# diegoferigo/gym-ignition

Hardware: AMD Instinct MI355X
Metric: env·steps/sec (whole node) at N parallel worlds; obs max-abs-err vs DART (higher is better)
Workload: dtype f32

## Files before the change

### gym-ignition_amd/csrc/vecenv_kernel.hip

```cpp
#include <cstdlib>
#include <type_traits>

#include "baked_models.hpp"
#include "chain_dyn.hpp"
#include "kernels.hpp"
#include "rng.hpp"

namespace mw {
namespace dev {

__constant__ constexpr baked::CartpoleBlock kCartpoleDev = {{MW_BAKED_CARTPOLE_INIT}};
__constant__ constexpr baked::PendulumBlock kPendulumDev = {{MW_BAKED_PENDULUM_INIT}};

template <int BAKED>
__device__ __forceinline__ const ChainF* model_params(const ChainF* P) {
    if constexpr (BAKED == baked::kCartpoleId) return reinterpret_cast<const ChainF*>(&kCartpoleDev);
    else if constexpr (BAKED == baked::kPendulumId) return reinterpret_cast<const ChainF*>(&kPendulumDev);
    else return P;
}

struct VecTail {
    float* obs;
    float* reward;
    uint8_t* done;
    float* term_obs;
    int32_t T_steps;
    int32_t max_steps;
    int32_t reward_cart_at_center;
    uint32_t seed_lo, seed_hi;
    uint32_t world_offset;
    float force_mag;
    float x_factor;
    float hi[4];
};
struct VecTailRand : VecTail {
    int32_t randomize;
    float mass_lo, mass_hi;
    float g_mean, g_std;
    float gdir[3];
    float* rmass;
    float* rgz;
};
template <bool RAND, bool GENERIC>
struct VecArgs : std::conditional_t<RAND, VecTailRand, VecTail> {};
template <bool RAND>
struct VecArgs<RAND, true> : std::conditional_t<RAND, VecTailRand, VecTail> {
    const ChainF* P;
};
static_assert(sizeof(VecArgs<true, true>) <= 136, "the step kernel's kernargs stay within 192 bytes");

template <class A>
__device__ __forceinline__ void fetch_now(const A& a) {
    static_assert(sizeof(A) % 4 == 0);
    uint32_t v[sizeof(A) / 4];
    __builtin_memcpy(v, &a, sizeof(A));
#pragma unroll
    for (unsigned k = 0; k < sizeof(A) / 4; ++k) asm volatile("" ::"s"(v[k]));
}

constexpr float kPi = 3.14159265358979323846f;

template <int N, int KIND, bool FOLD = false, class TT>
__device__ __forceinline__ void task_reset(const TT& T, uint32_t w, uint32_t episode,
                                           float (&q)[N], float (&qd)[N]) {
    uint32_t r[4];
    philox(T.seed_lo, T.seed_hi, w, episode, r);
    const auto unif = [](uint32_t x, float lo, float hi) {
        if constexpr (FOLD) return unif_folded(x, lo, hi);
        else return dev::unif(x, lo, hi);
    };
    if constexpr (KIND == 0 || KIND == 1) {
        q[0] = unif(r[0], -0.05f, 0.05f); qd[0] = unif(r[1], -0.05f, 0.05f);
        q[1] = unif(r[2], -0.05f, 0.05f); qd[1] = unif(r[3], -0.05f, 0.05f);
    } else if constexpr (KIND == 2) {
        q[1] = kPi - unif(r[0], -60.f, 60.f) * (kPi / 180.f);
        q[0] = unif(r[1], -0.05f, 0.05f); qd[0] = unif(r[2], -0.05f, 0.05f);
        qd[1] = unif(r[3], -0.05f, 0.05f);
    } else {
        const float c = unif(r[0], -1.f, 1.f), s = unif(r[1], -1.f, 1.f);
        q[0] = atan2f(s, c);
        qd[0] = unif(r[2], -10.f, 10.f);
    }
}

template <int N, int KIND>
__device__ __forceinline__ void task_obs(const float (&q)[N], const float (&qd)[N], float (&o)[4]) {
    if constexpr (KIND == 3) {
        float s, c;
        sincosf(q[0], &s, &c);
        o[0] = c; o[1] = s; o[2] = qd[0]; o[3] = 0.f;
    } else {
        o[0] = q[0]; o[1] = qd[0]; o[2] = q[1]; o[3] = qd[1];
    }
}

template <int KIND, bool ABS = false, class TT>
__device__ __forceinline__ bool task_done(const TT& T, const float (&o)[4]) {
    constexpr int no = (KIND == 3) ? 3 : 4;
    bool inside = true;
#pragma unroll
    for (int k = 0; k < no; ++k) {
        if constexpr (ABS) inside = inside & (fabsf(o[k]) <= T.hi[k]);
        else inside = inside & (o[k] >= -T.hi[k]) & (o[k] <= T.hi[k]);
    }
    return !inside;
}

template <int N, int KIND, class TT>
__device__ __forceinline__ float task_reward(const TT& T, const float (&q)[N], const float (&qd)[N],
                                             const float (&o)[4], bool done) {
#pragma clang fp contract(off)
    if constexpr (KIND == 0 || KIND == 1) {
        float r = done ? 0.f : 1.f;
        if (T.reward_cart_at_center)
            r = r - 0.10f * fabsf(o[0]) - 0.10f * fabsf(o[1]) -
                10.0f * (o[0] >= T.x_factor * 2.4f ? 1.f : 0.f);
        return r;
    } else if constexpr (KIND == 2) {
        return (cosf(q[1]) + 1.f) * 0.5f - 0.1f * qd[0] * qd[0] -
               10.0f * (q[0] >= T.x_factor * 2.4f ? 1.f : 0.f);
    } else {
        const float cost = (done ? 100.f : 0.f) + q[0] * q[0] + 0.1f * qd[0] * qd[0];
        return -cost;
    }
}

template <int N, class TT>
__device__ __forceinline__ Dyn<N> sample_dyn(const ChainF* __restrict__ P, const TT& T, uint32_t w,
                                             uint32_t episode, float& gz_out) {
    Dyn<N> D = nominal_dyn<N>(P);
    gz_out = 0.f;
    if (T.randomize & kRandMass) {
#pragma unroll
        for (int b = 0; b < (N + 3) / 4; ++b) {
            uint32_t r[4];
            philox(T.seed_lo, T.seed_hi, w, episode, r, 1u + static_cast<uint32_t>(b));
#pragma unroll
            for (int k = 0; k < 4; ++k)
                if (4 * b + k < N) D.m[4 * b + k] += fmaxf(unif(r[k], T.mass_lo, T.mass_hi), 0.f);
        }
    }
    if (T.randomize & kRandGravity) {
        uint32_t r[4];
        philox(T.seed_lo, T.seed_hi, w, episode, r, 8u);
        const float u1 = static_cast<float>((r[0] >> 8) + 1u) * (1.f / 16777216.f);
        const float u2 = static_cast<float>(r[1] >> 8) * (1.f / 16777216.f);
        const float z = sqrtf(-2.f * logf(u1)) * cosf(2.f * kPi * u2);
        const float gz = T.g_mean + T.g_std * z;
        D.g = {gz * T.gdir[0], gz * T.gdir[1], gz * T.gdir[2]};
        gz_out = gz;
    }
    return D;
}

template <int N, class TT, class VV>
__device__ __forceinline__ Dyn<N> load_dyn(const ChainF* __restrict__ P, const TT& T, const VV& V, int W, int w) {
    Dyn<N> D = nominal_dyn<N>(P);
    if (T.randomize & kRandMass) {
#pragma unroll
        for (int d = 0; d < N; ++d) D.m[d] = V.rmass[d * W + w];
    }
    if (T.randomize & kRandGravity) {
        const float gz = V.rgz[w];
        D.g = {gz * T.gdir[0], gz * T.gdir[1], gz * T.gdir[2]};
    }
    return D;
}

template <int N, class TT, class VV>
__device__ __forceinline__ void store_dyn(const TT& T, const VV& V, int W, int w, const Dyn<N>& D, float gz) {
    if (T.randomize & kRandMass) {
#pragma unroll
        for (int d = 0; d < N; ++d) V.rmass[d * W + w] = D.m[d];
    }
    if (T.randomize & kRandGravity) V.rgz[w] = gz;
}

template <bool OFF32, class E, class I>
__device__ __forceinline__ E* elem(E* base, I i) {
    if constexpr (OFF32) {
        using Byte = std::conditional_t<std::is_const_v<E>, const char, char>;
        return reinterpret_cast<E*>(reinterpret_cast<Byte*>(base) +
                                    static_cast<uint32_t>(i) * static_cast<uint32_t>(sizeof(E)));
    } else {
        return base + i;
    }
}

__device__ __forceinline__ int own_block(int w) {
    asm volatile("" : "+v"(w));
    return w;
}

template <int N, bool OFF32 = false>
__device__ __forceinline__ void store_state(float* __restrict__ sq, float* __restrict__ sqd, int W, int w,
                                            const float (&q)[N], const float (&qd)[N]) {
#pragma unroll
    for (int d = 0; d < N; ++d) {
        *elem<OFF32>(sq, d * W + w) = q[d];
        *elem<OFF32>(sqd, d * W + w) = qd[d];
    }
}

template <int NO>
__device__ __forceinline__ void store_obs(float* __restrict__ dst, const float (&o)[4]) {
    if constexpr (NO == 4) {
        *reinterpret_cast<float4*>(dst) = make_float4(o[0], o[1], o[2], o[3]);
    } else {
#pragma unroll
        for (int k = 0; k < NO; ++k) dst[k] = o[k];
    }
}


template <int N, int KIND>
__global__ void __launch_bounds__(256) vecenv_reset_kernel(const ChainF* __restrict__ P, TaskF T, SimDev S,
                                                           VecDev V, float* __restrict__ obs, int W) {
    const int w = blockIdx.x * blockDim.x + threadIdx.x;
    if (w >= W) return;
    float q[N], qd[N], o[4];
    if (T.randomize) {
        const uint32_t gw = T.world_offset + static_cast<uint32_t>(w);
        float gz;
        const Dyn<N> D = sample_dyn<N>(P, T, gw, 0u, gz);
        store_dyn<N>(T, V, W, w, D, gz);
    }
    task_reset<N, KIND>(T, T.world_offset + static_cast<uint32_t>(w), 0u, q, qd);
    task_obs<N, KIND>(q, qd, o);
    constexpr int NO = (KIND == 3) ? 3 : 4;
    store_obs<NO>(obs + static_cast<size_t>(w) * NO, o);
    store_state<N>(S.q, S.qd, W, w, q, qd);
    V.episode[w] = 0u;
    V.steps[w] = 0u;
}

constexpr int kHelpMaxWorlds = 64 * 256;
template <int N, int KIND, bool DUAL, bool CONS, bool ROLLOUT, int BAKED, bool RAND, int B, bool HELP = false,
          bool ONE = false>
__global__ void __launch_bounds__(256) vecenv_step_kernel(float* __restrict__ sq, float* __restrict__ sqd,
                                                          uint32_t* __restrict__ ep, uint32_t* __restrict__ st,
                                                          const void* __restrict__ actions, int W, float dt,
                                                          int substeps, int pgs_iters,
                                                          VecArgs<RAND, BAKED == 0> A) {
    static_assert(!HELP || (B == 64 && !ROLLOUT && !RAND), "the helper wave serves the closed-loop 64-world blocks");
    static_assert(!ONE || HELP, "the single-substep form exists for the helper-wave kernels");
    static_assert(static_cast<uint64_t>(kHelpMaxWorlds) * (N > 4 ? N : 4) * sizeof(float) < (1ull << 32),
                  "32-bit byte offsets cover every array of the HELP kernels");
    __shared__ float reset_lds[HELP ? 2 * N * B : 1];
    const int lane = HELP ? static_cast<int>(threadIdx.x) & (B - 1) : static_cast<int>(threadIdx.x);
    int w = blockIdx.x * B + lane;
    bool live = true;
    if constexpr (HELP) {
        live = w < W;
        w = live ? w : W - 1;
    } else {
        if (w >= W) return;
    }
    constexpr int NO = (KIND == 3) ? 3 : 4;
    using ActT = std::conditional_t<KIND == 0, int32_t, float>;
    float q[N], qd[N];
#pragma unroll
    for (int d = 0; d < N; ++d) {
        q[d] = *elem<HELP>(sq, d * W + w);
        qd[d] = *elem<HELP>(sqd, d * W + w);
    }
    const uint32_t episode0 = *elem<HELP>(ep, w);
    uint32_t episode = episode0;
    uint32_t steps = *elem<HELP>(st, w);
    ActT a0 = ActT(0);
    if constexpr (!ROLLOUT) a0 = *elem<HELP>(static_cast<const ActT*>(actions), w);
    fetch_now(A);
    float* __restrict__ obs = A.obs;
    float* __restrict__ reward = A.reward;
    uint8_t* __restrict__ done_out = A.done;
    float* __restrict__ term_obs = A.term_obs;
    const ChainF* __restrict__ P;
    if constexpr (BAKED == 0) P = A.P;
    else P = model_params<BAKED>(nullptr);
    uint8_t act[N];
    float vc[N];
#pragma unroll
    for (int d = 0; d < N; ++d) { act[d] = kActForce; vc[d] = 0.f; }
    Dyn<N> D;
    if constexpr (RAND) D = load_dyn<N>(P, A, A, W, w);
    if constexpr (HELP) {
        if (__builtin_amdgcn_readfirstlane(static_cast<int>(threadIdx.x)) >= B) {
            float rq[N], rqd[N];
            task_reset<N, KIND, true>(A, A.world_offset + static_cast<uint32_t>(w), episode0 + 1u, rq, rqd);
#pragma unroll
            for (int d = 0; d < N; ++d) {
                reset_lds[d * B + lane] = rq[d];
                reset_lds[(N + d) * B + lane] = rqd[d];
            }
            __syncthreads();
#pragma unroll
            for (int d = 0; d < N; ++d) asm volatile("" ::"v"(q[d]), "v"(qd[d]));
            asm volatile("" ::"v"(steps), "v"(a0));
            return;
        }
    }
    int ws = w;
    const int nsteps = ROLLOUT ? A.T_steps : 1;
    for (int t = 0; t < nsteps; ++t) {
        const size_t idx = static_cast<size_t>(t) * W + w;
        ActT a = a0;
        if constexpr (ROLLOUT) a = static_cast<const ActT*>(actions)[idx];
        float force;
        if constexpr (KIND == 0) {
            force = (a == 1) ? A.force_mag : -A.force_mag;
        } else {
            force = a;
        }
        const float e = P->b[0].effort;
        force = fminf(fmaxf(force, -e), e);
        float tau[N], qdd[N];
        if constexpr (ONE) {
#pragma unroll
            for (int d = 0; d < N; ++d) tau[d] = 0.f;
            tau[0] = force;
            substep<N, DUAL, CONS>(P, q, qd, tau, act, vc, dt, pgs_iters, qdd);
        } else {
            for (int s = 0; s < substeps; ++s) {
#pragma unroll
                for (int d = 0; d < N; ++d) tau[d] = 0.f;
                tau[0] = (s == 0) ? force : 0.f;
                if constexpr (RAND) substep_dyn<N, DUAL, CONS>(P, q, qd, tau, act, vc, dt, pgs_iters, qdd, D);
                else substep<N, DUAL, CONS>(P, q, qd, tau, act, vc, dt, pgs_iters, qdd);
            }
        }
        if constexpr (!ROLLOUT) asm volatile("" ::"v"(a0));
        float o[4];
        task_obs<N, KIND>(q, qd, o);
        const bool tdone = task_done<KIND, HELP>(A, o);
        const float rew = task_reward<N, KIND>(A, q, qd, o, tdone);
        if constexpr (!HELP) reward[idx] = rew;
        steps += 1u;
        const bool d_ = tdone || (A.max_steps > 0 && steps >= static_cast<uint32_t>(A.max_steps));
        if constexpr (HELP) {
            __syncthreads();
            if (!live) return;
            *elem<HELP>(reward, idx) = rew;
        }
        if constexpr (HELP) *elem<true>(done_out, idx) = d_ ? 1 : 0;
        else done_out[idx] = d_ ? 1 : 0;
        if (d_) {
            if constexpr (HELP) store_obs<NO>(elem<true>(term_obs, own_block(w) * NO), o);
            else store_obs<NO>(term_obs + idx * NO, o);
            episode += 1u;
            steps = 0u;
            if constexpr (RAND) {
                float gz;
                D = sample_dyn<N>(P, A, A.world_offset + static_cast<uint32_t>(w), episode, gz);
                store_dyn<N>(A, A, W, w, D, gz);
            }
            if constexpr (HELP) {
#pragma unroll
                for (int d = 0; d < N; ++d) {
                    q[d] = reset_lds[d * B + lane];
                    qd[d] = reset_lds[(N + d) * B + lane];
                }
            } else {
                task_reset<N, KIND>(A, A.world_offset + static_cast<uint32_t>(w), episode, q, qd);
            }
            task_obs<N, KIND>(q, qd, o);
        }
        if constexpr (HELP) {
            ws = own_block(w);
            store_obs<NO>(elem<true>(obs, ws * NO), o);
        } else {
            store_obs<NO>(obs + idx * NO, o);
        }
    }
    store_state<N, HELP>(sq, sqd, W, ws, q, qd);
    if constexpr (HELP) {
        *elem<true>(st, ws) = steps;
        if (episode != episode0) *elem<true>(ep, own_block(ws)) = episode;
    } else {
        if (episode != episode0) ep[w] = episode;
        st[w] = steps;
    }
}

}

namespace {

dim3 grid_for(int W, int block) { return dim3(static_cast<unsigned>((W + block - 1) / block)); }

int block_for(int W) { return (W <= dev::kHelpMaxWorlds) ? 64 : 256; }

bool substep_loop_forced() {
    const char* v = std::getenv("MWSTEP_FORCE_SUBSTEP_LOOP");
    return v && *v && *v != '0';
}

struct StepCall {
    const ChainF* P;
    const TaskF& T;
    const SimDev& S;
    const VecDev& V;
    const void* a;
    float *o, *r;
    uint8_t* d;
    float* to;
    int W;
    float dt;
    int substeps, pgs, Ts;
    hipStream_t st;
};

template <bool RAND, bool GENERIC>
dev::VecArgs<RAND, GENERIC> step_args(const StepCall& c) {
    dev::VecArgs<RAND, GENERIC> A;
    const TaskF& T = c.T;
    A.obs = c.o; A.reward = c.r; A.done = c.d; A.term_obs = c.to;
    A.T_steps = c.Ts;
    A.max_steps = T.max_steps;
    A.reward_cart_at_center = T.reward_cart_at_center;
    A.seed_lo = T.seed_lo; A.seed_hi = T.seed_hi;
    A.world_offset = T.world_offset;
    A.force_mag = T.force_mag;
    A.x_factor = T.x_factor;
    for (int k = 0; k < 4; ++k) A.hi[k] = T.hi[k];
    if constexpr (RAND) {
        A.randomize = T.randomize;
        A.mass_lo = T.mass_lo; A.mass_hi = T.mass_hi;
        A.g_mean = T.g_mean; A.g_std = T.g_std;
        for (int k = 0; k < 3; ++k) A.gdir[k] = T.gdir[k];
        A.rmass = c.V.rmass; A.rgz = c.V.rgz;
    }
    if constexpr (GENERIC) A.P = c.P;
    return A;
}

template <int N, int KIND, bool DUAL, bool CONS, bool ROLLOUT, int BAKED, bool RAND>
hipError_t vec_launch(const StepCall& c) {
    const auto A = step_args<RAND, BAKED == 0>(c);
    const int W = c.W;
    constexpr bool HELP = !ROLLOUT && !RAND;
    if (HELP && block_for(W) == 64 && c.substeps == 1 && !substep_loop_forced())
        hipLaunchKernelGGL((dev::vecenv_step_kernel<N, KIND, DUAL, CONS, ROLLOUT, BAKED, RAND, 64, HELP, HELP>),
                           grid_for(W, 64), dim3(128), 0, c.st, c.S.q, c.S.qd, c.V.episode, c.V.steps, c.a, W, c.dt,
                           c.substeps, c.pgs, A);
    else if (block_for(W) == 64)
        hipLaunchKernelGGL((dev::vecenv_step_kernel<N, KIND, DUAL, CONS, ROLLOUT, BAKED, RAND, 64, HELP>),
                           grid_for(W, 64), dim3(HELP ? 128 : 64), 0, c.st, c.S.q, c.S.qd, c.V.episode, c.V.steps, c.a,
                           W, c.dt, c.substeps, c.pgs, A);
    else
        hipLaunchKernelGGL((dev::vecenv_step_kernel<N, KIND, DUAL, CONS, ROLLOUT, BAKED, RAND, 256>), grid_for(W, 256),
                           dim3(256), 0, c.st, c.S.q, c.S.qd, c.V.episode, c.V.steps, c.a, W, c.dt, c.substeps, c.pgs,
                           A);
    return hipGetLastError();
}

template <int N, int KIND, bool ROLLOUT, bool RAND>
hipError_t vec_nk(bool cons, bool dual, int baked, const StepCall& c) {
    if constexpr (N == 2 && KIND <= 2) {
        if (baked == baked::kCartpoleId && cons && !dual)
            return vec_launch<N, KIND, false, true, ROLLOUT, baked::kCartpoleId, RAND>(c);
    }
    if constexpr (N == 1 && KIND == 3) {
        if (baked == baked::kPendulumId && !cons)
            return vec_launch<N, KIND, false, false, ROLLOUT, baked::kPendulumId, RAND>(c);
    }
    if (!cons) return vec_launch<N, KIND, false, false, ROLLOUT, 0, RAND>(c);
    if (!dual) return vec_launch<N, KIND, false, true, ROLLOUT, 0, RAND>(c);
    return vec_launch<N, KIND, true, true, ROLLOUT, 0, RAND>(c);
}

}

hipError_t launch_vecenv_reset(const ChainF* P, int n, const TaskF& T, const SimDev& S,
                               const VecDev& V, float* obs, int W, hipStream_t st) {
    if (T.kind == 4) return launch_vecenv_pid_reset(P, n, T, S, V, obs, W, st);
    const int B = block_for(W);
    if (T.kind == 3 && n == 1)
        hipLaunchKernelGGL((dev::vecenv_reset_kernel<1, 3>), grid_for(W, B), dim3(B), 0, st, P, T, S, V, obs, W);
    else if (T.kind == 0 && n == 2)
        hipLaunchKernelGGL((dev::vecenv_reset_kernel<2, 0>), grid_for(W, B), dim3(B), 0, st, P, T, S, V, obs, W);
    else if (T.kind == 1 && n == 2)
        hipLaunchKernelGGL((dev::vecenv_reset_kernel<2, 1>), grid_for(W, B), dim3(B), 0, st, P, T, S, V, obs, W);
    else if (T.kind == 2 && n == 2)
        hipLaunchKernelGGL((dev::vecenv_reset_kernel<2, 2>), grid_for(W, B), dim3(B), 0, st, P, T, S, V, obs, W);
    else
        return hipErrorInvalidValue;
    return hipGetLastError();
}

hipError_t launch_vecenv_step(const ChainF* P, int n, bool cons, bool dual, int baked, const TaskF& T,
                              const SimDev& S, const VecDev& V, const void* actions, float* obs,
                              float* reward, uint8_t* done, float* term_obs, int W, float dt,
                              int substeps, int pgs_iters, int T_steps, hipStream_t st) {
    const StepCall c{P, T, S, V, actions, obs, reward, done, term_obs, W, dt, substeps, pgs_iters,
                     T_steps > 0 ? T_steps : 1, st};
#define MW_VEC_R(NN, KK, RR) \
    return (T_steps > 0) ? vec_nk<NN, KK, true, RR>(cons, dual, baked, c) : vec_nk<NN, KK, false, RR>(cons, dual, baked, c)
#define MW_VEC(NN, KK)              \
    if (T.randomize) MW_VEC_R(NN, KK, true); \
    MW_VEC_R(NN, KK, false)
    if (T.kind == 3 && n == 1) { MW_VEC(1, 3); }
    if (T.kind == 0 && n == 2) { MW_VEC(2, 0); }
    if (T.kind == 1 && n == 2) { MW_VEC(2, 1); }
    if (T.kind == 2 && n == 2) { MW_VEC(2, 2); }
#undef MW_VEC
#undef MW_VEC_R
    return hipErrorInvalidValue;
}

}
```

### gym-ignition_amd/csrc/group_kernel.hip

```cpp
#include "group_tree.hpp"
#include "kernels.hpp"
#include "rng.hpp"
#include "xcd.hpp"

namespace mw {
namespace dev {

#ifdef MW_GROUP_PROF
__device__ unsigned long long g_group_prof[kGroupProfPhases];
#endif

template <int N, bool DUAL, bool CONS>
__global__ void __launch_bounds__(64) vecenv_pid_group_kernel(const ChainF* __restrict__ P, TaskF T, SimDev S,
                                                              VecDev V, const GLaneTask* __restrict__ lt,
                                                              const float* __restrict__ targets,
                                                              float* __restrict__ obs, float* __restrict__ reward,
                                                              uint8_t* __restrict__ done_out,
                                                              float* __restrict__ term_obs, int W, int n, float dt,
                                                              float inv_dt, int substeps, int pgs_iters) {
    unsigned long long prof[kGroupProfPhases] = {};
    MW_GPROF_T(k0);
    const int li = static_cast<int>(threadIdx.x) & (kGroupLanes - 1);
    const int wb = xcd_block();
    const int wr = static_cast<int>((wb * blockDim.x + threadIdx.x) / kGroupLanes);
    const bool live = wr < W;
    const int w = live ? wr : W - 1;
    const bool body = li < n;
    const GBody<N> B = load_gbody<N>(P, li, n);
    const GTopo TT = load_gtopo(P);
    PidF g{};
    float home = 0.f;
    if (body) {
        g = lt[li].pid;
        home = lt[li].home;
    }
    const f3 grav = {P->g[0], P->g[1], P->g[2]};
    const int dl = body ? li : 0;
    float q = 0.f, qd = 0.f, qlo = 0.f, tgt = 0.f, pe = 0.f, pi = 0.f, pu = 0.f;
    if (body) {
        q = S.q[dl * W + w];
        qd = S.qd[dl * W + w];
        qlo = S.qlo[dl * W + w];
        tgt = targets[static_cast<size_t>(w) * n + dl];
        pe = S.pid_e[dl * W + w];
        pi = S.pid_i[dl * W + w];
        pu = S.pid_u[dl * W + w];
    }
    const uint32_t episode0 = V.episode[w];
    const uint32_t steps0 = V.steps[w];
    MW_GPROF_T(k1);
    MW_GPROF_ACC(0, k0, k1);
    for (int s = 0; s < substeps; ++s) {
        float tau = 0.f;
        if (body) {
            float u = pu;
            if (!pid_update(g, (q - tgt) + qlo, inv_dt, dt, pe, pi, u)) u = 0.f;
            else pu = u;
            tau = fminf(fmaxf(u, -B.effort), B.effort);
        }
        group_substep<N, DUAL, CONS>(B, li, n, TT, grav, q, qd, qlo, tau, dt, inv_dt, pgs_iters,
                                     prof);
    }
    MW_GPROF_T(k2);
    const float e = body ? (q - tgt) * (q - tgt) : 0.f;
    float r = 0.f;
    sfor<N>([&](auto D) { r -= row_bcast<D>(e); });
    uint32_t steps = steps0 + 1u;
    const bool d_ = (T.max_steps > 0 && steps >= static_cast<uint32_t>(T.max_steps));
    if (live && li == 0) {
        reward[w] = r;
        done_out[w] = d_ ? 1 : 0;
    }
    const size_t ob = static_cast<size_t>(w) * 2 * n;
    if (d_) {
        if (live && body) {
            term_obs[ob + li] = q;
            term_obs[ob + n + li] = qd;
        }
        steps = 0u;
        if (live && li == 0) V.episode[w] = episode0 + 1u;
        uint32_t rr[4];
        philox(T.seed_lo, T.seed_hi, T.world_offset + static_cast<uint32_t>(w), episode0 + 1u, rr,
               static_cast<uint32_t>(li >> 2));
        const int k = li & 3;
        const uint32_t x4 = (k == 0) ? rr[0] : (k == 1) ? rr[1] : (k == 2) ? rr[2] : rr[3];
        const float x = home + unif(x4, -T.home_noise, T.home_noise);
        q = B.limited ? fminf(fmaxf(x, B.lower), B.upper) : x;
        qd = 0.f;
        pe = pi = pu = qlo = 0.f;
    }
    if (live && body) {
        obs[ob + li] = q;
        obs[ob + n + li] = qd;
        S.q[dl * W + w] = q;
        S.qd[dl * W + w] = qd;
        S.qlo[dl * W + w] = qlo;
        S.pid_e[dl * W + w] = pe;
        S.pid_i[dl * W + w] = pi;
        S.pid_u[dl * W + w] = pu;
    }
    if (live && li == 0) V.steps[w] = steps;
#ifdef MW_GROUP_PROF
    MW_GPROF_T(k3);
    MW_GPROF_ACC(7, k2, k3);
    MW_GPROF_ACC(8, k0, k3);
    if (live && li == 0)
        for (int k = 0; k < kGroupProfPhases; ++k) atomicAdd(&g_group_prof[k], prof[k]);
#else
    (void)prof;
#endif
}

}

#ifdef MW_GROUP_PROF
extern "C" int mw_debug_group_prof(unsigned long long* out) {
    if (hipMemcpyFromSymbol(out, HIP_SYMBOL(dev::g_group_prof), sizeof(dev::g_group_prof)) != hipSuccess) return 1;
    const unsigned long long z[dev::kGroupProfPhases] = {};
    return hipMemcpyToSymbol(HIP_SYMBOL(dev::g_group_prof), z, sizeof(z)) == hipSuccess ? 0 : 1;
}
#endif

namespace {
template <int N>
hipError_t group_n(const ChainF* P, int n, bool cons, bool dual, const TaskF& T, const SimDev& S, const VecDev& V,
                   const GLaneTask* pid, const float* targets, float* obs, float* reward, uint8_t* done, float* term_obs,
                   int W, float dt, int substeps, int pgs, hipStream_t st) {
    const dim3 grid(static_cast<unsigned>((W + 3) / 4)), block(64);
    const float inv_dt = 1.f / dt;
    if (!cons)
        hipLaunchKernelGGL((dev::vecenv_pid_group_kernel<N, false, false>), grid, block, 0, st, P, T, S, V, pid,
                           targets, obs, reward, done, term_obs, W, n, dt, inv_dt, substeps, pgs);
    else if (!dual)
        hipLaunchKernelGGL((dev::vecenv_pid_group_kernel<N, false, true>), grid, block, 0, st, P, T, S, V, pid,
                           targets, obs, reward, done, term_obs, W, n, dt, inv_dt, substeps, pgs);
    else
        hipLaunchKernelGGL((dev::vecenv_pid_group_kernel<N, true, true>), grid, block, 0, st, P, T, S, V, pid,
                           targets, obs, reward, done, term_obs, W, n, dt, inv_dt, substeps, pgs);
    return hipGetLastError();
}
}

hipError_t launch_vecenv_pid_group(const ChainF* P, int n, bool cons, bool dual, const TaskF& T, const SimDev& S,
                                   const VecDev& V, const GLaneTask* pid, const float* targets, float* obs,
                                   float* reward, uint8_t* done, float* term_obs, int W, float dt, int substeps,
                                   int pgs_iters, hipStream_t st) {
    if (n < 1 || n > kMaxKernelDofs || W < 1) return hipErrorInvalidValue;
    if (n <= 9)
        return group_n<9>(P, n, cons, dual, T, S, V, pid, targets, obs, reward, done, term_obs, W, dt, substeps,
                          pgs_iters, st);
    return group_n<kMaxKernelDofs>(P, n, cons, dual, T, S, V, pid, targets, obs, reward, done, term_obs, W, dt,
                                   substeps, pgs_iters, st);
}

}
```

### gym-ignition_amd/csrc/group_tree.hpp

```cpp
#pragma once

#include <hip/hip_runtime.h>

#include <utility>

#include "chain_dyn.hpp"
#include "pid.hpp"

namespace mw {
namespace dev {

constexpr int kGroupLanes = 16;
constexpr int kGroupMaxBodies = kGroupLanes;

constexpr int kGroupProfPhases = 10;
#ifdef MW_GROUP_PROF
#define MW_GPROF_T(var) const long long var = clock64()
#define MW_GPROF_ACC(k, a, b) (prof[k] += static_cast<unsigned long long>((b) - (a)))
#else
#define MW_GPROF_T(var)
#define MW_GPROF_ACC(k, a, b)
#endif

template <int K>
__device__ __forceinline__ float row_bcast(float x) {
    return __int_as_float(__builtin_amdgcn_update_dpp(0, __float_as_int(x), 0x150 + K, 0xf, 0xf, false));
}
template <int K>
__device__ __forceinline__ int row_bcast_i(int x) {
    return __builtin_amdgcn_update_dpp(0, x, 0x150 + K, 0xf, 0xf, false);
}
template <int S>
__device__ __forceinline__ float row_down(float x) {
    return __int_as_float(__builtin_amdgcn_update_dpp(0, __float_as_int(x), 0x100 + S, 0xf, 0xf, true));
}
template <int S>
__device__ __forceinline__ float row_up(float x) {
    return __int_as_float(__builtin_amdgcn_update_dpp(0, __float_as_int(x), 0x110 + S, 0xf, 0xf, true));
}
__device__ __forceinline__ float row_shfl(float x, int src) { return __shfl(x, src, kGroupLanes); }
__device__ __forceinline__ int row_shfl(int x, int src) { return __shfl(x, src, kGroupLanes); }

template <class F, int... I>
__device__ __forceinline__ void sfor_(F&& f, std::integer_sequence<int, I...>) {
    (f(std::integral_constant<int, I>{}), ...);
}
template <int N, class F>
__device__ __forceinline__ void sfor(F&& f) {
    sfor_(f, std::make_integer_sequence<int, N>{});
}

__device__ __forceinline__ float row_suffix(float x) {
    x += row_down<1>(x);
    x += row_down<2>(x);
    x += row_down<4>(x);
    x += row_down<8>(x);
    return x;
}

template <int N>
struct GBody {
    M3 E;
    f3 r, axis, com, Ea;
    Sy Icm;
    float mass, damping, friction, lower, upper, effort;
    int prism, limited, parent;
    int end;
    int hp, level;
    float bodyf;
    float seg[4];
    float eq[N], ge[N], anc[N];
};

template <int N>
__device__ __forceinline__ GBody<N> load_gbody(const ChainF* __restrict__ P, int li, int n) {
    GBody<N> g{};
    const bool body = li < n;
    const BodyF& b = P->b[body ? li : 0];
    const float bf = body ? 1.f : 0.f;
#pragma unroll
    for (int k = 0; k < 9; ++k) g.E.m[k] = body ? b.E[k] : ((k % 4 == 0) ? 1.f : 0.f);
    g.r = bf * f3{b.r[0], b.r[1], b.r[2]};
    g.axis = bf * f3{b.axis[0], b.axis[1], b.axis[2]};
    g.com = bf * f3{b.com[0], b.com[1], b.com[2]};
    g.Ea = bf * f3{b.Ea[0], b.Ea[1], b.Ea[2]};
    const float m = bf * b.mass, cx = b.com[0], cy = b.com[1], cz = b.com[2];
    g.Icm = {bf * b.Io[0] - m * (cy * cy + cz * cz), bf * b.Io[1] - m * (cx * cx + cz * cz),
             bf * b.Io[2] - m * (cx * cx + cy * cy), bf * b.Io[3] + m * cx * cy, bf * b.Io[4] + m * cx * cz,
             bf * b.Io[5] + m * cy * cz};
    g.mass = m;
    g.damping = bf * b.damping;
    g.friction = bf * b.friction;
    g.lower = b.lower;
    g.upper = b.upper;
    g.effort = b.effort;
    g.prism = body ? (b.jtype & 1) : 0;
    g.limited = body ? b.limited : 0;
    g.parent = body ? b.parent : -1;
    const uint32_t anc = body ? b.anc : 0u;
    g.end = body ? b.end : li + 1;
    const int seg = body ? b.seg : 0;
    const int h = seg & 0xff;
    g.hp = ((seg >> 8) & 0xff) - 1;
    g.level = (seg >> 16) & 0xff;
    g.bodyf = bf;
    g.seg[0] = h >= 1 ? 1.f : 0.f;
    g.seg[1] = h >= 2 ? 1.f : 0.f;
    g.seg[2] = h >= 4 ? 1.f : 0.f;
    g.seg[3] = h >= 8 ? 1.f : 0.f;
#pragma unroll
    for (int k = 0; k < N; ++k) {
        g.eq[k] = (li == k) ? 1.f : 0.f;
        g.ge[k] = (li >= k) ? 1.f : 0.f;
        g.anc[k] = ((anc >> k) & 1u) ? 1.f : 0.f;
    }
    return g;
}

struct GTopo {
    int steps, levels, ref;
    int fix;
    int dend;
    bool diff;
};
__device__ __forceinline__ GTopo load_gtopo(const ChainF* __restrict__ P) {
    const int a = P->gtopo, b = P->gtopo2;
    return {(a >> 16) & 0xff, (a >> 8) & 0xff, a & 0xff, (b & 0xff) - 1, ((b >> 8) & 0xff) - 1, ((b >> 16) & 1) != 0};
}

template <class F>
__device__ __forceinline__ void with_lane(int k, F&& f) {
    sfor<kGroupLanes>([&](auto K) {
        if (k == K) f(K);
    });
}

template <int K, int N>
__device__ __forceinline__ void tree_prefix(float (&x)[K], const GBody<N>& B, const GTopo& T, int li) {
    auto step = [&](auto S) {
        constexpr int s = S;
        constexpr int e = (s == 1) ? 0 : (s == 2) ? 1 : (s == 4) ? 2 : 3;
#pragma unroll
        for (int k = 0; k < K; ++k) x[k] = fmaf(row_up<s>(x[k]), B.seg[e], x[k]);
    };
    if (T.steps > 0) step(std::integral_constant<int, 1>{});
    if (T.steps > 1) step(std::integral_constant<int, 2>{});
    if (T.steps > 2) step(std::integral_constant<int, 4>{});
    if (T.steps > 3) step(std::integral_constant<int, 8>{});
    if (T.fix >= 0) {
        const float fm = (B.level == 1) ? 1.f : 0.f;
        with_lane(T.fix, [&](auto L) {
#pragma unroll
            for (int k = 0; k < K; ++k) x[k] = fmaf(row_bcast<L>(x[k]), fm, x[k]);
        });
        return;
    }
    for (int r = 1; r <= T.levels; ++r) {
        const bool fix = B.level == r;
        const float fm = fix ? 1.f : 0.f;
        const int src = fix ? B.hp : li;
#pragma unroll
        for (int k = 0; k < K; ++k) x[k] = fmaf(row_shfl(x[k], src), fm, x[k]);
    }
}

__device__ __forceinline__ void compose_masked(M3 Ra, f3 pa, float m, M3& R, f3& p) {
    const float m1 = 1.f - m;
#pragma unroll
    for (int k = 0; k < 9; ++k) Ra.m[k] *= m;
    Ra.m[0] += m1; Ra.m[4] += m1; Ra.m[8] += m1;
    pa = m * pa;
    p = mul(Ra, p) + pa;
    M3 Rn;
#pragma unroll
    for (int r = 0; r < 3; ++r)
#pragma unroll
        for (int k = 0; k < 3; ++k)
            Rn.m[r * 3 + k] = Ra.m[r * 3] * R.m[k] + Ra.m[r * 3 + 1] * R.m[3 + k] + Ra.m[r * 3 + 2] * R.m[6 + k];
    R = Rn;
}
template <int N>
__device__ __forceinline__ void tree_poses(M3& R, f3& p, const GBody<N>& B, const GTopo& T, int li) {
    auto step = [&](auto S) {
        constexpr int s = S;
        constexpr int e = (s == 1) ? 0 : (s == 2) ? 1 : (s == 4) ? 2 : 3;
        M3 Ra;
#pragma unroll
        for (int k = 0; k < 9; ++k) Ra.m[k] = row_up<s>(R.m[k]);
        const f3 pa = {row_up<s>(p.x), row_up<s>(p.y), row_up<s>(p.z)};
        compose_masked(Ra, pa, B.seg[e], R, p);
    };
    if (T.steps > 0) step(std::integral_constant<int, 1>{});
    if (T.steps > 1) step(std::integral_constant<int, 2>{});
    if (T.steps > 2) step(std::integral_constant<int, 4>{});
    if (T.steps > 3) step(std::integral_constant<int, 8>{});
    if (T.fix >= 0) {
        with_lane(T.fix, [&](auto L) {
            M3 Ra;
#pragma unroll
            for (int k = 0; k < 9; ++k) Ra.m[k] = row_bcast<L>(R.m[k]);
            const f3 pa = {row_bcast<L>(p.x), row_bcast<L>(p.y), row_bcast<L>(p.z)};
            compose_masked(Ra, pa, (B.level == 1) ? 1.f : 0.f, R, p);
        });
        return;
    }
    for (int r = 1; r <= T.levels; ++r) {
        const bool fix = B.level == r;
        const int src = fix ? B.hp : li;
        M3 Ra;
#pragma unroll
        for (int k = 0; k < 9; ++k) Ra.m[k] = row_shfl(R.m[k], src);
        const f3 pa = {row_shfl(p.x, src), row_shfl(p.y, src), row_shfl(p.z, src)};
        compose_masked(Ra, pa, fix ? 1.f : 0.f, R, p);
    }
}

template <int K>
__device__ __forceinline__ void subtree_sum(float (&x)[K], int end, int li, const GTopo& T) {
#pragma unroll
    for (int k = 0; k < K; ++k) x[k] = row_suffix(x[k]);
    if (T.dend >= 0) {
        const float sm = (end == T.dend) ? 1.f : 0.f;
        with_lane(T.dend, [&](auto L) {
#pragma unroll
            for (int k = 0; k < K; ++k) x[k] = fmaf(-row_bcast<L>(x[k]), sm, x[k]);
        });
    } else if (T.diff) {
        const bool sub = end < kGroupLanes;
        const float sm = sub ? 1.f : 0.f;
        const int src = sub ? end : li;
#pragma unroll
        for (int k = 0; k < K; ++k) x[k] = fmaf(-row_shfl(x[k], src), sm, x[k]);
    }
}

template <int N>
struct RowChol {
    float r[N], ct[N], inv[N];
};

template <int N, int M>
__device__ __forceinline__ void row_factor(RowChol<N>& C, const GBody<M>& B) {
    sfor<N>([&](auto K) {
        constexpr int k = K;
        const float dk = row_bcast<k>(C.r[k]);
        const float ik = __builtin_amdgcn_rsqf(dk);
        C.inv[k] = ik;
        const float lik = C.r[k] * ik;
        C.r[k] = lik;
        sfor<N - k - 1>([&](auto J) {
            constexpr int j = k + 1 + J;
            const float ljk = row_bcast<j>(lik);
            C.r[j] = fmaf(-lik, ljk, C.r[j]);
            C.ct[j] = fmaf(B.eq[k], ljk, C.ct[j]);
        });
    });
}

template <int N, int K0 = 0, int M>
__device__ __forceinline__ float row_solve(const RowChol<N>& C, float b, const GBody<M>& B) {
    float y = 0.f;
    sfor<N - K0>([&](auto KK) {
        constexpr int k = K0 + KK;
        const float yk = row_bcast<k>(b) * C.inv[k];
        y = fmaf(B.eq[k], yk, y);
        b = fmaf(-C.r[k], yk, b);
    });
    float x = 0.f;
    sfor<N>([&](auto KK) {
        constexpr int k = N - 1 - KK;
        const float xk = row_bcast<k>(y) * C.inv[k];
        x = fmaf(B.eq[k], xk, x);
        y = fmaf(-C.ct[k], xk, y);
    });
    return x;
}

struct GI {
    float m;
    f3 h;
    Sy J;
};
__device__ __forceinline__ SV gmul(const GI& I, const SV& V) {
    return {mul(I.J, V.w) + cross(I.h, V.v), I.m * V.v - cross(I.h, V.w)};
}

template <int N, bool DUAL, bool CONS>
__device__ __forceinline__ void group_substep(const GBody<N>& B, int li, int n, const GTopo& T,
                                              f3 grav, float& q, float& qd, float& qlo, float tau, float dt,
                                              float inv_dt, int pgs_iters,
                                              unsigned long long (&prof)[kGroupProfPhases]) {
    (void)prof;
    (void)n;
    MW_GPROF_T(t0);
    M3 R;
    f3 p;
    if (!B.prism) {
        float s, c;
        sincos_joint(q, &s, &c);
        const float ax = B.axis.x, ay = B.axis.y, az = B.axis.z, v = 1.f - c;
        const float J[9] = {c + ax * ax * v,      ax * ay * v - az * s, ax * az * v + ay * s,
                            ay * ax * v + az * s, c + ay * ay * v,      ay * az * v - ax * s,
                            az * ax * v - ay * s, az * ay * v + ax * s, c + az * az * v};
#pragma unroll
        for (int r = 0; r < 3; ++r)
#pragma unroll
            for (int k = 0; k < 3; ++k)
                R.m[r * 3 + k] = B.E.m[r * 3] * J[k] + B.E.m[r * 3 + 1] * J[3 + k] + B.E.m[r * 3 + 2] * J[6 + k];
        p = B.r;
    } else {
        R = B.E;
        p = B.r + q * B.Ea;
    }
    tree_poses(R, p, B, T, li);
    {
        f3 pr = {0.f, 0.f, 0.f};
        with_lane(T.ref, [&](auto K) { pr = {row_bcast<K>(p.x), row_bcast<K>(p.y), row_bcast<K>(p.z)}; });
        p = p - pr;
    }
    MW_GPROF_T(t1);
    MW_GPROF_ACC(1, t0, t1);
    const f3 a0 = mul(R, B.axis);
    SV S;
    if (!B.prism) S = {a0, cross(p, a0)};
    else S = {{0.f, 0.f, 0.f}, a0};
    GI I;
    {
        const f3 c0 = mul(R, B.com) + p;
        const Sy Jr = rot_sym(R, B.Icm);
        const float m = B.mass, cc = dot(c0, c0);
        I.m = m;
        I.h = m * c0;
        I.J = {Jr.xx + m * (cc - c0.x * c0.x), Jr.yy + m * (cc - c0.y * c0.y), Jr.zz + m * (cc - c0.z * c0.z),
               Jr.xy - m * c0.x * c0.y,        Jr.xz - m * c0.x * c0.z,        Jr.yz - m * c0.y * c0.z};
    }
    float ci[10] = {I.m, I.h.x, I.h.y, I.h.z, I.J.xx, I.J.yy, I.J.zz, I.J.xy, I.J.xz, I.J.yz};
    subtree_sum<10>(ci, B.end, li, T);
    const GI Ic = {ci[0], {ci[1], ci[2], ci[3]}, {ci[4], ci[5], ci[6], ci[7], ci[8], ci[9]}};
    const SV F = gmul(Ic, S);
    RowChol<N> C;
    RowChol<(DUAL && CONS) ? N : 1> Cn;
    {
        const float diag = fmaf(B.bodyf, dot(S, F) - 1.f, 1.f);
        const float diag_i = diag + dt * B.damping;
        sfor<N>([&](auto J) {
            constexpr int j = J;
            float mij = 0.f;
            if constexpr (j < N - 1) {
                const SV Sj = {{row_bcast<j>(S.w.x), row_bcast<j>(S.w.y), row_bcast<j>(S.w.z)},
                               {row_bcast<j>(S.v.x), row_bcast<j>(S.v.y), row_bcast<j>(S.v.z)}};
                mij = B.anc[j] * dot(Sj, F);
            }
            C.r[j] = fmaf(B.eq[j], diag_i, mij);
            if constexpr (DUAL && CONS) Cn.r[j] = fmaf(B.eq[j], diag, mij);
            C.ct[j] = 0.f;
            C.inv[j] = 0.f;
            if constexpr (DUAL && CONS) { Cn.ct[j] = 0.f; Cn.inv[j] = 0.f; }
        });
    }
    MW_GPROF_T(t2);
    MW_GPROF_ACC(2, t1, t2);
    float hb;
    {
        const SV Sq = qd * S;
        float v6[6] = {Sq.w.x, Sq.w.y, Sq.w.z, Sq.v.x, Sq.v.y, Sq.v.z};
        tree_prefix<6>(v6, B, T, li);
        const SV V = {{v6[0], v6[1], v6[2]}, {v6[3], v6[4], v6[5]}};
        const SV cv = {cross(V.w, Sq.w), cross(V.w, Sq.v) + cross(V.v, Sq.w)};
        float a6[6] = {cv.w.x, cv.w.y, cv.w.z, cv.v.x, cv.v.y, cv.v.z};
        tree_prefix<6>(a6, B, T, li);
        const SV A = {{a6[0], a6[1], a6[2]}, {a6[3] - grav.x, a6[4] - grav.y, a6[5] - grav.z}};
        const SV IV = gmul(I, V);
        const SV IA = gmul(I, A);
        float f6[6];
        {
            const f3 fw = IA.w + cross(V.w, IV.w) + cross(V.v, IV.v);
            const f3 fv = IA.v + cross(V.w, IV.v);
            f6[0] = fw.x; f6[1] = fw.y; f6[2] = fw.z; f6[3] = fv.x; f6[4] = fv.y; f6[5] = fv.z;
        }
        subtree_sum<6>(f6, B.end, li, T);
        hb = dot(S, SV{{f6[0], f6[1], f6[2]}, {f6[3], f6[4], f6[5]}});
    }
    MW_GPROF_T(t3);
    MW_GPROF_ACC(3, t2, t3);
    row_factor<N>(C, B);
    const float rhs = B.bodyf * (tau - B.damping * qd - hb);
    float qdd = row_solve<N>(C, rhs, B);
    qd += dt * qdd;
    MW_GPROF_T(t4);
    MW_GPROF_ACC(4, t3, t4);

    if constexpr (CONS) {
        uint32_t on = 0u;
        bool up = false;
        float b0 = 0.f, b2 = 0.f;
        if (B.limited) {
            float viol = q - B.lower;
            bool act = false;
            if (viol <= 0.f) {
                act = true;
            } else {
                viol = q - B.upper;
                if (viol >= 0.f) { act = true; up = true; }
            }
            if (act) {
                on |= 1u;
                const float bounce = fminf(fmaxf(-viol * kErp * inv_dt, -kMaxErv), kMaxErv);
                b0 = -qd + bounce;
            }
        }
        if (B.friction != 0.f && qd != 0.f) { on |= 4u; b2 = -qd; }
        if (__any(on != 0u)) {
            if constexpr (DUAL) row_factor<N>(Cn, B);
            float mc[N], invd[N], rb0[N], rb2[N], lo0[N], hi0[N], a0m[N], a2m[N], x0[N], x2[N];
            auto rows_of = [](uint64_t m) {
                return static_cast<uint32_t>((m | (m >> 16) | (m >> 32) | (m >> 48)) & 0xffffu);
            };
            const uint32_t rows0 = rows_of(__ballot((on & 1u) != 0u));
            const uint32_t rows2 = rows_of(__ballot((on & 4u) != 0u));
            const float onf0 = (on & 1u) ? 1.f : 0.f, onf2 = (on & 4u) ? 1.f : 0.f, upf = up ? 1.f : 0.f;
            sfor<N>([&](auto D) {
                constexpr int d = D;
                x0[d] = x2[d] = 0.f;
                mc[d] = invd[d] = rb0[d] = rb2[d] = a0m[d] = a2m[d] = lo0[d] = hi0[d] = 0.f;
                if (((rows0 | rows2) >> d) & 1u) {
                    rb0[d] = row_bcast<d>(b0);
                    rb2[d] = row_bcast<d>(b2);
                    a0m[d] = row_bcast<d>(onf0);
                    a2m[d] = row_bcast<d>(onf2);
                    const float u = row_bcast<d>(upf);
                    lo0[d] = u != 0.f ? -kBig : 0.f;
                    hi0[d] = u != 0.f ? 0.f : kBig;
                    if constexpr (DUAL) mc[d] = row_solve<N, d>(Cn, B.eq[d], B);
                    else mc[d] = row_solve<N, d>(C, B.eq[d], B);
                    invd[d] = rcp(row_bcast<d>(mc[d]));
                }
            });
            MW_GPROF_T(t5);
            MW_GPROF_ACC(5, t4, t5);
            float dq = 0.f;
            for (int it = 0; it < pgs_iters; ++it) {
                float moved = 0.f;
                sfor<N>([&](auto D) {
                    constexpr int d = D;
                    if ((rows0 >> d) & 1u) {
                        const float xn = fminf(fmaxf(x0[d] + (rb0[d] - row_bcast<d>(dq)) * invd[d], lo0[d]), hi0[d]);
                        const float delta = (xn - x0[d]) * a0m[d];
                        moved = fmaxf(moved, fabsf(delta));
                        x0[d] += delta;
                        dq = fmaf(delta, mc[d], dq);
                    }
                    if ((rows2 >> d) & 1u) {
                        const float fr = row_bcast<d>(B.friction) * dt;
                        const float xn = fminf(fmaxf(x2[d] + (rb2[d] - row_bcast<d>(dq)) * invd[d], -fr), fr);
                        const float delta = (xn - x2[d]) * a2m[d];
                        moved = fmaxf(moved, fabsf(delta));
                        x2[d] += delta;
                        dq = fmaf(delta, mc[d], dq);
                    }
                });
#ifdef MW_GROUP_PROF
                prof[9] += 1;
#endif
                if (!__any(moved != 0.f)) break;
            }
            qd += dq;
            qdd += dq * inv_dt;
            MW_GPROF_T(t6);
            MW_GPROF_ACC(6, t5, t6);
        }
    }
    const float h = dt * qd;
    const float s = q + h;
    const float bv = s - q;
    const float err = (q - (s - bv)) + (h - bv);
    const float lo = qlo + err;
    const float hi = s + lo;
    qlo = lo - (hi - s);
    q = hi;
    (void)qdd;
}

}
}
```

Measured before the change: 1.975 billion.

## Extend helper-wave speculative reset to randomized-dynamics worlds with mass/gravity draw waves

Closed-loop step kernels with domain randomization now use the helper-wave layout. Four waves per 64-world block replace one. Wave 0 steps the physics, wave 1 precomputes the next reset state, and waves 2 and 3 pre-draw the next episode's randomized masses and gravity into LDS. The compute wave reads the current per-world dynamics directly and, on episode end, copies the pre-drawn values from LDS instead of sampling them inline. This keeps RNG and reset latency off the critical path, at the cost of 4x threads per block, more LDS, and a barrier. An env var restores the inline-draw path.

```diff
diff --git a/gym-ignition_amd/csrc/vecenv_kernel.hip b/gym-ignition_amd/csrc/vecenv_kernel.hip
--- a/gym-ignition_amd/csrc/vecenv_kernel.hip
+++ b/gym-ignition_amd/csrc/vecenv_kernel.hip
@@ -242,11 +242,11 @@
                                                           const void* __restrict__ actions, int W, float dt,
                                                           int substeps, int pgs_iters,
                                                           VecArgs<RAND, BAKED == 0> A) {
-    static_assert(!HELP || (B == 64 && !ROLLOUT && !RAND), "the helper wave serves the closed-loop 64-world blocks");
+    static_assert(!HELP || (B == 64 && !ROLLOUT), "the helper waves serve the closed-loop 64-world blocks");
     static_assert(!ONE || HELP, "the single-substep form exists for the helper-wave kernels");
     static_assert(static_cast<uint64_t>(kHelpMaxWorlds) * (N > 4 ? N : 4) * sizeof(float) < (1ull << 32),
                   "32-bit byte offsets cover every array of the HELP kernels");
-    __shared__ float reset_lds[HELP ? 2 * N * B : 1];
+    __shared__ float reset_lds[HELP ? (RAND ? 3 * N + 1 : 2 * N) * B : 1];
     const int lane = HELP ? static_cast<int>(threadIdx.x) & (B - 1) : static_cast<int>(threadIdx.x);
     int w = blockIdx.x * B + lane;
     bool live = true;
@@ -270,6 +270,12 @@
     ActT a0 = ActT(0);
     if constexpr (!ROLLOUT) a0 = *elem<HELP>(static_cast<const ActT*>(actions), w);
     fetch_now(A);
+    float lm[N], lgz = 0.f;
+    if constexpr (HELP && RAND) {
+#pragma unroll
+        for (int d = 0; d < N; ++d) lm[d] = *elem<true>(A.rmass, d * W + w);
+        lgz = *elem<true>(A.rgz, w);
+    }
     float* __restrict__ obs = A.obs;
     float* __restrict__ reward = A.reward;
     uint8_t* __restrict__ done_out = A.done;
@@ -282,8 +288,16 @@
 #pragma unroll
     for (int d = 0; d < N; ++d) { act[d] = kActForce; vc[d] = 0.f; }
     Dyn<N> D;
-    if constexpr (RAND) D = load_dyn<N>(P, A, A, W, w);
-    if constexpr (HELP) {
+    if constexpr (HELP && RAND) {
+        D = nominal_dyn<N>(P);
+        const bool rm = A.randomize & kRandMass, rg = A.randomize & kRandGravity;
+#pragma unroll
+        for (int d = 0; d < N; ++d) D.m[d] = rm ? lm[d] : D.m[d];
+        D.g = {rg ? lgz * A.gdir[0] : D.g.x, rg ? lgz * A.gdir[1] : D.g.y, rg ? lgz * A.gdir[2] : D.g.z};
+    } else if constexpr (RAND) {
+        D = load_dyn<N>(P, A, A, W, w);
+    }
+    if constexpr (HELP && !RAND) {
         if (__builtin_amdgcn_readfirstlane(static_cast<int>(threadIdx.x)) >= B) {
             float rq[N], rqd[N];
             task_reset<N, KIND, true>(A, A.world_offset + static_cast<uint32_t>(w), episode0 + 1u, rq, rqd);
@@ -297,6 +311,43 @@
             for (int d = 0; d < N; ++d) asm volatile("" ::"v"(q[d]), "v"(qd[d]));
             asm volatile("" ::"v"(steps), "v"(a0));
             return;
+        }
+    }
+    if constexpr (HELP && RAND) {
+        const int role = __builtin_amdgcn_readfirstlane(static_cast<int>(threadIdx.x)) / B;
+        if (__builtin_expect(role != 0, true)) {
+            const uint32_t gw = A.world_offset + static_cast<uint32_t>(w);
+            if (role == 1) {
+                float rq[N], rqd[N];
+                task_reset<N, KIND, true>(A, gw, episode0 + 1u, rq, rqd);
+#pragma unroll
+                for (int d = 0; d < N; ++d) {
+                    reset_lds[d * B + lane] = rq[d];
+                    reset_lds[(N + d) * B + lane] = rqd[d];
+                }
+            } else if (role == 2) {
+                if (A.randomize & kRandMass) {
+                    VecTailRand part = A;
+                    part.randomize = kRandMass;
+                    float gz;
+                    const Dyn<N> Dn = sample_dyn<N>(P, part, gw, episode0 + 1u, gz);
+#pragma unroll
+                    for (int d = 0; d < N; ++d) reset_lds[(2 * N + d) * B + lane] = Dn.m[d];
+                }
+            } else {
+                if (A.randomize & kRandGravity) {
+                    VecTailRand part = A;
+                    part.randomize = kRandGravity;
+                    float gz;
+                    sample_dyn<N>(P, part, gw, episode0 + 1u, gz);
+                    reset_lds[3 * N * B + lane] = gz;
+                }
+            }
+            __syncthreads();
+#pragma unroll
+            for (int d = 0; d < N; ++d) asm volatile("" ::"v"(q[d]), "v"(qd[d]), "v"(lm[d]));
+            asm volatile("" ::"v"(steps), "v"(a0), "v"(lgz));
+            __builtin_amdgcn_endpgm();
         }
     }
     int ws = w;
@@ -318,7 +369,8 @@
 #pragma unroll
             for (int d = 0; d < N; ++d) tau[d] = 0.f;
             tau[0] = force;
-            substep<N, DUAL, CONS>(P, q, qd, tau, act, vc, dt, pgs_iters, qdd);
+            if constexpr (RAND) substep_dyn<N, DUAL, CONS>(P, q, qd, tau, act, vc, dt, pgs_iters, qdd, D);
+            else substep<N, DUAL, CONS>(P, q, qd, tau, act, vc, dt, pgs_iters, qdd);
         } else {
             for (int s = 0; s < substeps; ++s) {
 #pragma unroll
@@ -348,7 +400,14 @@
             else store_obs<NO>(term_obs + idx * NO, o);
             episode += 1u;
             steps = 0u;
-            if constexpr (RAND) {
+            if constexpr (HELP && RAND) {
+                const int wd = own_block(w);
+                if (A.randomize & kRandMass) {
+#pragma unroll
+                    for (int d = 0; d < N; ++d) *elem<true>(A.rmass, d * W + wd) = reset_lds[(2 * N + d) * B + lane];
+                }
+                if (A.randomize & kRandGravity) *elem<true>(A.rgz, wd) = reset_lds[3 * N * B + lane];
+            } else if constexpr (RAND) {
                 float gz;
                 D = sample_dyn<N>(P, A, A.world_offset + static_cast<uint32_t>(w), episode, gz);
                 store_dyn<N>(A, A, W, w, D, gz);
@@ -391,6 +450,11 @@
 
 bool substep_loop_forced() {
     const char* v = std::getenv("MWSTEP_FORCE_SUBSTEP_LOOP");
+    return v && *v && *v != '0';
+}
+
+bool inline_draws_forced() {
+    const char* v = std::getenv("MWSTEP_FORCE_INLINE_DRAWS");
     return v && *v && *v != '0';
 }
 
@@ -437,14 +501,25 @@
 hipError_t vec_launch(const StepCall& c) {
     const auto A = step_args<RAND, BAKED == 0>(c);
     const int W = c.W;
-    constexpr bool HELP = !ROLLOUT && !RAND;
-    if (HELP && block_for(W) == 64 && c.substeps == 1 && !substep_loop_forced())
+    constexpr bool HELP = !ROLLOUT;
+    constexpr unsigned kThreads = RAND ? 256 : 128;
+    bool help = HELP;
+    if constexpr (RAND) help = help && !inline_draws_forced();
+    if constexpr (!HELP || RAND) {
+        if (!help && block_for(W) == 64) {
+            hipLaunchKernelGGL((dev::vecenv_step_kernel<N, KIND, DUAL, CONS, ROLLOUT, BAKED, RAND, 64>),
+                               grid_for(W, 64), dim3(64), 0, c.st, c.S.q, c.S.qd, c.V.episode, c.V.steps, c.a, W, c.dt,
+                               c.substeps, c.pgs, A);
+            return hipGetLastError();
+        }
+    }
+    if (block_for(W) == 64 && c.substeps == 1 && !substep_loop_forced())
         hipLaunchKernelGGL((dev::vecenv_step_kernel<N, KIND, DUAL, CONS, ROLLOUT, BAKED, RAND, 64, HELP, HELP>),
-                           grid_for(W, 64), dim3(128), 0, c.st, c.S.q, c.S.qd, c.V.episode, c.V.steps, c.a, W, c.dt,
+                           grid_for(W, 64), dim3(kThreads), 0, c.st, c.S.q, c.S.qd, c.V.episode, c.V.steps, c.a, W, c.dt,
                            c.substeps, c.pgs, A);
     else if (block_for(W) == 64)
         hipLaunchKernelGGL((dev::vecenv_step_kernel<N, KIND, DUAL, CONS, ROLLOUT, BAKED, RAND, 64, HELP>),
-                           grid_for(W, 64), dim3(HELP ? 128 : 64), 0, c.st, c.S.q, c.S.qd, c.V.episode, c.V.steps, c.a,
+                           grid_for(W, 64), dim3(kThreads), 0, c.st, c.S.q, c.S.qd, c.V.episode, c.V.steps, c.a,
                            W, c.dt, c.substeps, c.pgs, A);
     else
         hipLaunchKernelGGL((dev::vecenv_step_kernel<N, KIND, DUAL, CONS, ROLLOUT, BAKED, RAND, 256>), grid_for(W, 256),
```

After: 1.945 billion. 1.5% lower.

## Solve one- or two-row joint-limit LCPs directly instead of PGS sweeps

Applied to the files above, without the earlier changes.

Adds a DIRECT path to the grouped substep. When a world has only limit rows active, at most two of them and no friction rows, the small LCP is solved in closed form: a single clamp, or an enumeration of the two-row active sets with a Schur complement. The PGS loop is then skipped for the wavefront when every world in it takes the direct path. This is on by default, with an environment variable that restores the sweeps. The cost is extra register pressure and a change in numerics relative to iterated PGS, which could shift error against DART.

```diff
diff --git a/gym-ignition_amd/csrc/group_kernel.hip b/gym-ignition_amd/csrc/group_kernel.hip
--- a/gym-ignition_amd/csrc/group_kernel.hip
+++ b/gym-ignition_amd/csrc/group_kernel.hip
@@ -1,3 +1,6 @@
+#include <cstdlib>
+#include <cstring>
+
 #include "group_tree.hpp"
 #include "kernels.hpp"
 #include "rng.hpp"
@@ -10,7 +13,7 @@
 __device__ unsigned long long g_group_prof[kGroupProfPhases];
 #endif
 
-template <int N, bool DUAL, bool CONS>
+template <int N, bool DUAL, bool CONS, bool DIRECT = false>
 __global__ void __launch_bounds__(64) vecenv_pid_group_kernel(const ChainF* __restrict__ P, TaskF T, SimDev S,
                                                               VecDev V, const GLaneTask* __restrict__ lt,
                                                               const float* __restrict__ targets,
@@ -58,8 +61,8 @@
             else pu = u;
             tau = fminf(fmaxf(u, -B.effort), B.effort);
         }
-        group_substep<N, DUAL, CONS>(B, li, n, TT, grav, q, qd, qlo, tau, dt, inv_dt, pgs_iters,
-                                     prof);
+        group_substep<N, DUAL, CONS, DIRECT>(B, li, n, TT, grav, q, qd, qlo, tau, dt, inv_dt, pgs_iters,
+                                             prof);
     }
     MW_GPROF_T(k2);
     const float e = body ? (q - tgt) * (q - tgt) : 0.f;
@@ -122,6 +125,11 @@
 #endif
 
 namespace {
+bool group_lcp_sweeps() {
+    const char* v = std::getenv("MWSTEP_GROUP_LCP");
+    return v && std::strcmp(v, "sweeps") == 0;
+}
+
 template <int N>
 hipError_t group_n(const ChainF* P, int n, bool cons, bool dual, const TaskF& T, const SimDev& S, const VecDev& V,
                    const GLaneTask* pid, const float* targets, float* obs, float* reward, uint8_t* done, float* term_obs,
@@ -131,7 +139,14 @@
     if (!cons)
         hipLaunchKernelGGL((dev::vecenv_pid_group_kernel<N, false, false>), grid, block, 0, st, P, T, S, V, pid,
                            targets, obs, reward, done, term_obs, W, n, dt, inv_dt, substeps, pgs);
-    else if (!dual)
+    else if (!group_lcp_sweeps()) {
+        if (!dual)
+            hipLaunchKernelGGL((dev::vecenv_pid_group_kernel<N, false, true, true>), grid, block, 0, st, P, T, S, V,
+                               pid, targets, obs, reward, done, term_obs, W, n, dt, inv_dt, substeps, pgs);
+        else
+            hipLaunchKernelGGL((dev::vecenv_pid_group_kernel<N, true, true, true>), grid, block, 0, st, P, T, S, V,
+                               pid, targets, obs, reward, done, term_obs, W, n, dt, inv_dt, substeps, pgs);
+    } else if (!dual)
         hipLaunchKernelGGL((dev::vecenv_pid_group_kernel<N, false, true>), grid, block, 0, st, P, T, S, V, pid,
                            targets, obs, reward, done, term_obs, W, n, dt, inv_dt, substeps, pgs);
     else
diff --git a/gym-ignition_amd/csrc/group_tree.hpp b/gym-ignition_amd/csrc/group_tree.hpp
--- a/gym-ignition_amd/csrc/group_tree.hpp
+++ b/gym-ignition_amd/csrc/group_tree.hpp
@@ -13,7 +13,7 @@
 constexpr int kGroupLanes = 16;
 constexpr int kGroupMaxBodies = kGroupLanes;
 
-constexpr int kGroupProfPhases = 10;
+constexpr int kGroupProfPhases = 13;
 #ifdef MW_GROUP_PROF
 #define MW_GPROF_T(var) const long long var = clock64()
 #define MW_GPROF_ACC(k, a, b) (prof[k] += static_cast<unsigned long long>((b) - (a)))
@@ -285,7 +285,7 @@
     return {mul(I.J, V.w) + cross(I.h, V.v), I.m * V.v - cross(I.h, V.w)};
 }
 
-template <int N, bool DUAL, bool CONS>
+template <int N, bool DUAL, bool CONS, bool DIRECT = false>
 __device__ __forceinline__ void group_substep(const GBody<N>& B, int li, int n, const GTopo& T,
                                               f3 grav, float& q, float& qd, float& qlo, float tau, float dt,
                                               float inv_dt, int pgs_iters,
@@ -416,9 +416,28 @@
             auto rows_of = [](uint64_t m) {
                 return static_cast<uint32_t>((m | (m >> 16) | (m >> 32) | (m >> 48)) & 0xffffu);
             };
-            const uint32_t rows0 = rows_of(__ballot((on & 1u) != 0u));
-            const uint32_t rows2 = rows_of(__ballot((on & 4u) != 0u));
-            const float onf0 = (on & 1u) ? 1.f : 0.f, onf2 = (on & 4u) ? 1.f : 0.f, upf = up ? 1.f : 0.f;
+            const uint64_t bal0 = __ballot((on & 1u) != 0u);
+            const uint32_t rows0 = rows_of(bal0);
+            const uint64_t bal2 = __ballot((on & 4u) != 0u);
+            const uint32_t rows2 = rows_of(bal2);
+            uint32_t bi = 0u, bj = 0u;
+            bool direct = false, two = false;
+            if constexpr (DIRECT) {
+                const int sh = static_cast<int>(threadIdx.x) & 48;
+                const uint32_t m0 = static_cast<uint32_t>(bal0 >> sh) & 0xffffu;
+                const uint32_t m2 = static_cast<uint32_t>(bal2 >> sh) & 0xffffu;
+                bi = m0 & (0u - m0);
+                bj = m0 ^ bi;
+                two = bj != 0u;
+                direct = m2 == 0u && m0 != 0u && (bj & (bj - 1u)) == 0u && pgs_iters > 0;
+            }
+#ifdef MW_GROUP_PROF
+            {
+                const bool rows = (((bal0 | bal2) >> (static_cast<int>(threadIdx.x) & 48)) & 0xffffu) != 0u;
+                prof[direct ? 10 : rows ? 11 : 12] += 1;
+            }
+#endif
+            const float onf0 = ((on & 1u) && !direct) ? 1.f : 0.f, onf2 = (on & 4u) ? 1.f : 0.f, upf = up ? 1.f : 0.f;
             sfor<N>([&](auto D) {
                 constexpr int d = D;
                 x0[d] = x2[d] = 0.f;
@@ -439,7 +458,55 @@
             MW_GPROF_T(t5);
             MW_GPROF_ACC(5, t4, t5);
             float dq = 0.f;
-            for (int it = 0; it < pgs_iters; ++it) {
+            float dqx = 0.f;
+            int iters = pgs_iters;
+            if constexpr (DIRECT) {
+                float mci = 0.f, mcj = 0.f, rbi = 0.f, rbj = 0.f, ivi = 0.f, ivj = 0.f;
+                float loi = 0.f, hii = 0.f, loj = 0.f, hij = 0.f, aij = 0.f, ajj = 0.f;
+                sfor<N>([&](auto D) {
+                    constexpr int d = D;
+                    if ((rows0 >> d) & 1u) {
+                        const float si = ((bi >> d) & 1u) ? 1.f : 0.f, sj = ((bj >> d) & 1u) ? 1.f : 0.f;
+                        const float cij = row_bcast<d>(mci);
+                        const float cdd = row_bcast<d>(mc[d]);
+                        aij = fmaf(sj, cij, aij);
+                        ajj = fmaf(sj, cdd, ajj);
+                        mcj = fmaf(sj, mc[d], mcj);
+                        rbj = fmaf(sj, rb0[d], rbj);
+                        ivj = fmaf(sj, invd[d], ivj);
+                        loj = fmaf(sj, lo0[d], loj);
+                        hij = fmaf(sj, hi0[d], hij);
+                        mci = fmaf(si, mc[d], mci);
+                        rbi = fmaf(si, rb0[d], rbi);
+                        ivi = fmaf(si, invd[d], ivi);
+                        loi = fmaf(si, lo0[d], loi);
+                        hii = fmaf(si, hi0[d], hii);
+                    }
+                });
+                const float xi1 = fminf(fmaxf((rbi - 0.f) * ivi, loi), hii);
+                float xi = xi1, xj = 0.f;
+                const float sgi = hii == 0.f ? -1.f : 1.f, sgj = hij == 0.f ? -1.f : 1.f;
+                const float xj1 = fminf(fmaxf(rbj * ivj, loj), hij);
+                const float l = aij * ivi;
+                const float sch = fmaf(-l, aij, ajj);
+                const float xjf = fminf(fmaxf(fmaf(-l, rbi, rbj) * (sch > 0.f ? rcp(sch) : 0.f), loj), hij);
+                const float xif = fminf(fmaxf(fmaf(-aij, xjf, rbi) * ivi, loi), hii);
+                const bool bb = sgi * rbi <= 0.f && sgj * rbj <= 0.f;
+                const bool fb = sgi * rbi >= 0.f && sgj * fmaf(-aij, xi1, rbj) <= 0.f;
+                const bool bf = sgj * rbj >= 0.f && sgi * fmaf(-aij, xj1, rbi) <= 0.f;
+                if (two) {
+                    xi = bb ? 0.f : fb ? xi1 : bf ? 0.f : xif;
+                    xj = bb ? 0.f : fb ? 0.f : bf ? xj1 : xjf;
+                }
+                dqx = fmaf(xi, mci, 0.f);
+                dqx = two ? fmaf(xj, mcj, dqx) : dqx;
+                if (pgs_iters > 1) {
+                    const bool at_i = ((bi >> li) & 1u) != 0u, at_j = ((bj >> li) & 1u) != 0u;
+                    dqx = (at_i && xi != 0.f) ? rbi : (at_j && xj != 0.f) ? rbj : dqx;
+                }
+                if (!__any((on != 0u) && !direct)) iters = 0;
+            }
+            for (int it = 0; it < iters; ++it) {
                 float moved = 0.f;
                 sfor<N>([&](auto D) {
                     constexpr int d = D;
@@ -464,11 +531,15 @@
 #endif
                 if (!__any(moved != 0.f)) break;
             }
+            if constexpr (DIRECT) dq = direct ? dqx : dq;
             qd += dq;
             qdd += dq * inv_dt;
             MW_GPROF_T(t6);
             MW_GPROF_ACC(6, t5, t6);
         }
+#ifdef MW_GROUP_PROF
+        else prof[12] += 1;
+#endif
     }
     const float h = dt * qd;
     const float s = q + h;
```

After: 1.925 billion before, 1.920 billion after. About the same (-0.3%).
